# nurturenature/jepsen-tigerbeetle

Measured on NVIDIA H100. Metric: configs explored/sec (time-to-verdict alongside) on 10k-op/32-client bank history, higher is better.
Workload: dtype int64

## Files before the change

### jepsen_tigerbeetle_b200/csrc/jtb_abi.cu

```cuda
#include <algorithm>
#include <chrono>
#include <cstdio>
#include <cstdlib>
#include <cstring>
#include <mutex>
#include <string>
#include <thread>
#include <type_traits>
#include <vector>

#include "jtb_wgl.cuh"
#include "jtb_level.cuh"
#include "jtb_scout.cuh"
#include "jtb_scans.cuh"
#include "jtb_table_bench.cuh"
#include "jtb_partition.cuh"
#include "jtb_monotonic.cuh"
#include "jtb_counter_bounds.cuh"
#include "jtb_transfer_lookups.cuh"
#include "jtb_read_explanations.cuh"
#include "jtb_read_gaps.cuh"

using namespace jtb;

// ... 61 lines not shown
    if (ensure(ctx, b, v.size() * sizeof(T) + 64)) return -1;
    if (!v.empty()) CK(cudaMemcpyAsync(b.p, v.data(), v.size() * sizeof(T), cudaMemcpyHostToDevice, ctx->stream));
    return 0;
}

template <typename F>
int dispatch_model_kw(jtb_ctx* ctx, int kind, int kw, F&& f) {
    using std::integral_constant;
    if (kind == JTB_MODEL_SET) return f(integral_constant<int, JTB_MODEL_SET>(), integral_constant<int, 2>());
    auto by_kw = [&](auto model) -> int {
        switch (kw) {
        case 2: return f(model, integral_constant<int, 2>());
        case 4: return f(model, integral_constant<int, 4>());
        case 8: return f(model, integral_constant<int, 8>());
        }
        ctx->err = "unsupported key width";
        return -1;
    };
    return kind == JTB_MODEL_BANK ? by_kw(integral_constant<int, JTB_MODEL_BANK>())
                                  : by_kw(integral_constant<int, JTB_MODEL_CAS_REGISTER>());
}

template <int MODEL, int KW>
int launch_wgl(jtb_ctx* ctx, const WglParams& p, int neg_ok, int grid, size_t smem) {
    auto k = p.eager_reads ? wgl_search_kernel<MODEL, KW, JTB_CTAS_EAGER, true> : wgl_search_kernel<MODEL, KW, JTB_CTAS_EXACT, false>;
    CK(cudaFuncSetAttribute(k, cudaFuncAttributeMaxDynamicSharedMemorySize, (int)smem));
    k<<<grid, WGL_THREADS, smem, ctx->stream>>>(p, neg_ok);
    CK(cudaGetLastError());
    return 0;
}

template <int MODEL, int KW>
int launch_level(jtb_ctx* ctx, const LvParams& p, int neg_ok, bool eager, int* grid_out) {
    constexpr int EW = KW + (MODEL == JTB_MODEL_BANK ? 4 : 0);
    const bool beam = p.beam_w != 0;
    const size_t smem = (beam ? sizeof(LvScratch<KW, EW, MODEL == JTB_MODEL_BANK, true>)
                              : sizeof(LvScratch<KW, EW, MODEL == JTB_MODEL_BANK, false>)) * LV_WARPS;
    const bool nk = !(MODEL == JTB_MODEL_BANK && !neg_ok);
    const void* k;
#define JTB_LVK(E, N, B) (const void*)level_search_kernel<MODEL, KW, E, (MODEL == JTB_MODEL_BANK ? N : true), B>
    if (beam) k = eager ? (nk ? JTB_LVK(true, true, true) : JTB_LVK(true, false, true)) : (nk ? JTB_LVK(false, true, true) : JTB_LVK(false, false, true));
    else k = eager ? (nk ? JTB_LVK(true, true, false) : JTB_LVK(true, false, false)) : (nk ? JTB_LVK(false, true, false) : JTB_LVK(false, false, false));
#undef JTB_LVK
    CK(cudaFuncSetAttribute(k, cudaFuncAttributeMaxDynamicSharedMemorySize, (int)smem));
    int per_sm = 0;
    CK(cudaOccupancyMaxActiveBlocksPerMultiprocessor(&per_sm, k, LV_THREADS, smem));
    if (per_sm < 1) { ctx->err = "level engine: the kernel does not fit on an SM"; return -1; }
    per_sm = std::min(per_sm, JTB_LV_CTAS);
    const int grid = ctx->opts.search_ctas ? std::min<int>((int)ctx->opts.search_ctas, ctx->n_sms * per_sm) : ctx->n_sms * per_sm;
    if (grid > 1024) { ctx->err = "level engine: more CTAs than barrier release words"; return -1; }
    *grid_out = grid;
    LvParams pp = p;
    void* args[] = {&pp};
    CK(cudaLaunchCooperativeKernel(k, dim3(grid), dim3(LV_THREADS), args, smem, ctx->stream));
    return 0;
}

int search_level(jtb_ctx* ctx, const jtb_model* m, const Prepared& P, int n_shards, const std::vector<int>& searchable,
                 const std::vector<uint64_t>& init_entries, Ctrl& hc, double& kernel_s, uint64_t& configs, uint64_t& probes,
                 uint32_t beam_w = 0) {
    const int KW = P.key_words;
    const bool bank = m->kind == JTB_MODEL_BANK;
    const int EW = KW + (bank ? 4 : 0);
    const bool eager = !(ctx->opts.flags & JTB_OPT_NO_EAGER_READS);
    size_t free_b = 0, total_b = 0;
    CK(cudaMemGetInfo(&free_b, &total_b));
    const size_t reserve = (size_t)4 << 30;
    const size_t avail = ctx->table.cap + ctx->lv_buf[0].cap + ctx->lv_buf[1].cap + (free_b > reserve ? free_b - reserve : 0);
    size_t table_bytes = ctx->opts.table_bytes ? ctx->opts.table_bytes
                         : (getenv("JTB_LV_TABLE_MB") ? (size_t)atoll(getenv("JTB_LV_TABLE_MB")) << 20 : (size_t)1 << 30);
    table_bytes = std::min(table_bytes, avail / 3);
    size_t buf_bytes = getenv("JTB_LV_BUF_MB") ? (size_t)atoll(getenv("JTB_LV_BUF_MB")) << 20 : (size_t)512 << 20;
    buf_bytes = std::max<size_t>(std::min(buf_bytes, avail / 3), init_entries.size() * 8 + 4096);
    auto slots_of = [&](size_t bytes) { uint64_t s = 1; while (s * 2 * KW * 8 <= bytes) s <<= 1; return s; };
    uint64_t table_slots = slots_of(std::max(table_bytes, ctx->table.cap));
    auto ensure_table = [&](uint64_t slots) -> int {
        const void* before = ctx->table.p;
        if (ensure(ctx, ctx->table, slots * KW * 8)) return -1;
        if (ctx->table.p != before) ctx->table_dirty = ~(size_t)0;
        return 0;
    };
    if (ensure_table(table_slots)) return -1;
    if (ensure(ctx, ctx->lv_buf[0], std::max(buf_bytes, ctx->lv_buf[0].cap)) || ensure(ctx, ctx->lv_buf[1], std::max(buf_bytes, ctx->lv_buf[1].cap)) ||
        ensure(ctx, ctx->lv_ctrl, sizeof(LvCtrl)))
        return -1;
    uint64_t buf_cap = std::min(ctx->lv_buf[0].cap, ctx->lv_buf[1].cap) / ((size_t)EW * 8);
    if (beam_w) {
        if (ensure(ctx, ctx->lv_aux[0], buf_cap * 4 + 64) || ensure(ctx, ctx->lv_aux[1], buf_cap * 4 + 64) ||
            ensure(ctx, ctx->lv_beam, sizeof(LvBeam)))
            return -1;
        std::vector<LvBeam> hb(1);
        std::memset(hb.data(), 0, sizeof(LvBeam));
        for (int k = 0; k < 3; ++k)
            for (int s = 0; s < LV_BEAM_SHARDS; ++s) { hb[0].min_crashed[k][s] = 0x7fffffff; hb[0].max_rank[k][s] = -1; }
        for (int s : searchable) { hb[0].min_crashed[0][s] = 0; hb[0].max_rank[0][s] = (int)P.rank_base[s]; }
        CK(cudaMemcpyAsync(ctx->lv_beam.p, hb.data(), sizeof(LvBeam), cudaMemcpyHostToDevice, ctx->stream));
        CK(cudaMemsetAsync(ctx->lv_aux[0].p, 0, init_entries.size() / EW * 4 + 64, ctx->stream));
        CK(cudaStreamSynchronize(ctx->stream));
    }
    CK(cudaMemsetAsync(ctx->table.p, 0, std::min(ctx->table_dirty, (size_t)table_slots * KW * 8), ctx->stream));
    ctx->table_dirty = 0;
    LvCtrl lc;
    std::memset(&lc, 0, sizeof lc);
    lc.n_undecided = (int)searchable.size();
    CK(cudaMemcpyAsync(ctx->lv_ctrl.p, &lc, sizeof lc, cudaMemcpyHostToDevice, ctx->stream));
    CK(cudaMemcpyAsync(ctx->lv_buf[0].p, init_entries.data(), init_entries.size() * 8, cudaMemcpyHostToDevice, ctx->stream));
    LvParams p{};
    p.rows = (const int32_t*)ctx->rows.p;
    p.classes = (const ClassRec*)ctx->classes.p;
    p.cls_inv_pos = (const int32_t*)ctx->cls_inv.p;
    p.ctrl = (LvCtrl*)ctx->lv_ctrl.p;
    p.shard_found = (int*)ctx->found.p;
    p.shard_max_rank = (int*)ctx->maxrank.p;
    p.row_words = P.row_words;
    p.sum_off = P.sum_off;
    p.n_shards = n_shards;
    p.max_configs = ctx->opts.max_configs;
    p.time_budget_ns = (unsigned long long)ctx->opts.time_budget_ms * 1000000ull;
    p.narrow_max = getenv("JTB_LV_NARROW") ? (uint32_t)atoi(getenv("JTB_LV_NARROW")) : (uint32_t)(LV_WARPS * 8);
    p.slots_per_config = getenv("JTB_LV_SPC") ? (uint32_t)std::max(2, atoi(getenv("JTB_LV_SPC"))) : 16u;
    p.min_slots = 1ull << 16;
    std::memset(&p.init, 0, sizeof p.init);
    p.init.n_in = searchable.size();
    p.init.epoch = 1;
    p.init.s_in = 0; p.init.s_out = 1; p.init.s_spare = 2;
    p.init.contig = 1;
    p.init.beam_thr = -1;
    p.init.beam_frac = 1024;
    p.beam_w = beam_w;
    p.aux[0] = (uint32_t*)ctx->lv_aux[0].p;
    p.aux[1] = (uint32_t*)ctx->lv_aux[1].p;
    p.beam = (LvBeam*)ctx->lv_beam.p;
    p.init.win = 0;
    CK(cudaEventRecord(ctx->ev0, ctx->stream));
    int attempts = 0, grid = 0;
    unsigned long long max_window = 0, max_width = 0, narrow_levels = 0, max_probe = 0;
    const double t_begin = now_s();
    for (;;) {
        ++attempts;
// ... 74 lines not shown
        CK(cudaFree(ctx->lv_buf[ii].p));
        ctx->lv_buf[ii] = grown;
        if (ensure(ctx, ctx->lv_buf[ii ^ 1], new_buf)) return -1;
        table_slots = slots_of(new_table);
        if (ensure_table(table_slots)) return -1;
        CK(cudaMemsetAsync(ctx->table.p, 0, (size_t)table_slots * KW * 8, ctx->stream));
        ctx->table_dirty = 0;
        buf_cap = new_buf / ((size_t)EW * 8);
        LvState r = lc.fin;
        r.stop = 0; r.cause = 0; r.boost = 0; r.attempt = 0; r.epoch = 1;
        r.s_in = 0; r.s_out = 1; r.s_spare = 2; r.contig = 1;
        p.init = r;
        const int undecided = lc.n_undecided;
        std::memset(&lc, 0, sizeof lc);
        lc.n_undecided = undecided;
        CK(cudaMemcpyAsync(ctx->lv_ctrl.p, &lc, sizeof lc, cudaMemcpyHostToDevice, ctx->stream));
    }
    CK(cudaEventRecord(ctx->ev1, ctx->stream));
    CK(cudaStreamSynchronize(ctx->stream));
    float ms = 0;
    CK(cudaEventElapsedTime(&ms, ctx->ev0, ctx->ev1));
    kernel_s = ms * 1e-3;
    configs = lc.fin.total;
    std::memset(&hc, 0, sizeof hc);
    hc.stop = lc.fin.stop;
    hc.cause = lc.fin.cause;
    hc.configs = lc.fin.total;
    hc.probes = probes;
    hc.n_undecided = lc.n_undecided;
    unsigned long long* st = ctx->stats;
    st[0] = configs; st[1] = probes; st[2] = lc.fin.level + 1; st[3] = max_width; st[4] = narrow_levels; st[5] = 0;
    st[6] = max_probe; st[7] = max_window; st[8] = (unsigned long long)grid; st[9] = buf_cap;
    st[10] = (unsigned long long)attempts; st[11] = (unsigned long long)(ms * 1e3);
    st[12] += init_entries.size() * 8 + sizeof(LvCtrl) + (size_t)n_shards * 4;
    st[13] = (unsigned long long)attempts * sizeof(LvCtrl) + (size_t)n_shards * 8;
    st[14] = (unsigned long long)attempts;
    st[19] = 1;
    return 0;
}

struct ScoutGuard {
    jtb_ctx* ctx;
    bool active = false;
    explicit ScoutGuard(jtb_ctx* c) : ctx(c) {}
    int stop() {
        if (!active) return 0;
        active = false;
        static const unsigned long long one = 1;
        cudaError_t e = cudaMemcpyAsync((unsigned long long*)ctx->sc_ctl.p + 1, &one, 8, cudaMemcpyHostToDevice, ctx->stream);
        if (e == cudaSuccess) e = cudaStreamSynchronize(ctx->scout_stream);
        if (e != cudaSuccess) { ctx->err = std::string("stopping the scouts: ") + cudaGetErrorString(e); return -1; }
        return 0;
    }
    ~ScoutGuard() { stop(); }
};

template <typename K>
int preload(jtb_ctx* ctx, K kernel) {
    cudaFuncAttributes a;
    CK(cudaFuncGetAttributes(&a, kernel));
    return 0;
}

template <int MODEL, int KW>
int preload_search(jtb_ctx* ctx, bool eager) {
    constexpr int EW = KW + (MODEL == JTB_MODEL_BANK ? 4 : 0);
    int rc = eager ? (preload(ctx, wgl_search_kernel<MODEL, KW, JTB_CTAS_EAGER, true>) | preload(ctx, wgl_scout_kernel<MODEL, KW, true>))
// ... 785 lines not shown
```

### jepsen_tigerbeetle_b200/csrc/jtb_expand.h

```cpp
#pragma once
#include <cstdint>

#include "jtb_prep.h"

#if defined(__CUDACC__)
#define JTB_HD __host__ __device__ __forceinline__
#else
#define JTB_HD inline
#endif

namespace jtb {

constexpr uint64_t XKEY_VALID = 1ull << 63;
constexpr uint32_t XRANK_MASK = 0x1fffffffu;

struct I4 {
    int32_t x, y, z, w;
};

JTB_HD I4 ld_i4(const int32_t* p) {
#if defined(__CUDA_ARCH__)
    const int4 v = __ldg(reinterpret_cast<const int4*>(p));
    return I4{v.x, v.y, v.z, v.w};
#else
// ... 55 lines not shown

    JTB_HD int load_header(const ExpandTables& T) {
        gj = (int)((w[0] >> 32) & XRANK_MASK);
        reg = (int32_t)(uint32_t)w[0];
        row = T.rows + (size_t)gj * T.row_words;
        const I4 h2 = ld_i4(row + 8);
        fr_pos = h2.x; shard = h2.y; gj_end = h2.z; cls_base = h2.w;
        return shard;
    }

    JTB_HD bool read_consistent(const I4& op, const int32_t* cell, uint32_t balhash) const {
        if constexpr (REG) {
            return op.y == JTB_NIL || op.y == reg;
        } else if constexpr (BANK) {
            if ((op.x & OP_HASHED) && (uint32_t)op.z != balhash) return false;
            const I4 lo = ld_i4(cell + 4), hi = ld_i4(cell + 8);
            const int care = op.y;
            bool ok = true;
            ok &= !(care & 1) || bal[0] == lo.x;
            ok &= !(care & 2) || bal[1] == lo.y;
            ok &= !(care & 4) || bal[2] == lo.z;
            ok &= !(care & 8) || bal[3] == lo.w;
            ok &= !(care & 16) || bal[4] == hi.x;
            ok &= !(care & 32) || bal[5] == hi.y;
            ok &= !(care & 64) || bal[6] == hi.z;
            ok &= !(care & 128) || bal[7] == hi.w;
            return ok;
        } else {
            const I4 nc = ld_i4(cell + 4);
            return (w[1] & u64_of(nc.z, nc.w)) == u64_of(nc.x, nc.y);
        }
    }

    JTB_HD void begin(const ExpandTables& T, bool alive) {
        (void)T;
        const I4 h3 = ld_i4(row + 12);
        const I4 h4 = ld_i4(row + 16);
        ncls = h3.x; rslot = h3.y;
        todo = 0; rd_ok = 0; cls_i = ncls;
        if (!alive) return;
        const uint64_t cand = u64_of(h3.z, h3.w) & ~w[1];
        const uint64_t rdm = u64_of(h4.x, h4.y);
        uint64_t rds = cand & rdm;
        uint32_t balhash = 0;
        if constexpr (BANK) {
            if (rds) {
#pragma unroll
                for (int i = 0; i < 8; ++i) balhash += (uint32_t)bal[i] * bank_hash_c(i);
            }
        }
        if constexpr (!SET) {
            const uint64_t fastm = T.sum_off ? (rds & u64_of(h4.z, h4.w)) : 0ull;
            if (fastm) {
                const int32_t* sum = row + T.sum_off;
                const int32_t want = BANK ? (int32_t)balhash : reg;
                uint64_t match = 0;
#if defined(__CUDA_ARCH__)
#pragma unroll 1
#endif
                for (int b = 0; b < 4; ++b) {
                    if (!((fastm >> (16 * b)) & 0xffffull)) continue;
                    uint32_t mm = 0;
#pragma unroll
                    for (int g = 0; g < 4; ++g) {
                        const I4 v = ld_i4(sum + 16 * b + 4 * g);
                        uint32_t m4 = (v.x == want) | ((v.y == want) << 1) | ((v.z == want) << 2) | ((v.w == want) << 3);
                        if constexpr (REG)
                            m4 |= (v.x == JTB_NIL) | ((v.y == JTB_NIL) << 1) | ((v.z == JTB_NIL) << 2) | ((v.w == JTB_NIL) << 3);
                        mm |= m4 << (4 * g);
                    }
                    match |= (uint64_t)mm << (16 * b);
                }
                match &= fastm;
                if constexpr (REG && !EAGER) { rd_ok |= match; match = 0; }
                rds = (rds & ~fastm) | match;
            }
        }
        uint32_t best_inv = 0xffffffffu;
        int best_t = -1;
// ... 122 lines not shown
```

### jepsen_tigerbeetle_b200/csrc/jtb_level.cuh

```cuda
#pragma once
#include "jtb_expand.h"
#include "jtb_wgl.cuh"

namespace jtb {

#ifndef JTB_LV_WARPS
#define JTB_LV_WARPS 8
#endif
#ifndef JTB_LV_CTAS
#define JTB_LV_CTAS 3
#endif
constexpr int LV_WARPS = JTB_LV_WARPS;
constexpr int LV_THREADS = LV_WARPS * 32;
constexpr int LV_STAGE = 64;
constexpr int LV_MAX_PROBE = 128;
constexpr int LV_CLS_WORDS = 8;
constexpr uint64_t LV_TAG_MASK = 0x3full << 56;
constexpr int64_t LV_MAX_RANKS = 1ll << 24;

constexpr int LV_NSEG = 64;
constexpr unsigned LV_F_DECIDED = 1, LV_F_GIVEUP = 2, LV_F_RETRY = 4;

struct LvSeg {
    alignas(128) unsigned long long n;
// ... 34 lines not shown
    unsigned long long max_probe_len, max_width, max_window, narrow_levels, retries, t0, t1;
    LvState fin;
    unsigned long long prof[16];
    unsigned long long prof_cta[1024][2];
    int trace[2048][6];
    alignas(128) LvRelease arrive[1024];
    alignas(128) LvRelease release[1024];
};

struct LvParams {
    const int32_t* rows;
    const ClassRec* classes;
    const int32_t* cls_inv_pos;
    uint64_t* table;
    uint64_t table_slots;
    uint64_t* buf[2];
    uint32_t* aux[2];
    LvBeam* beam;
    uint32_t beam_w;
    uint64_t buf_cap;
    uint64_t seg_cap;
    LvCtrl* ctrl;
    int* shard_found;
    int* shard_max_rank;
    int row_words, sum_off, n_shards;
    unsigned long long max_configs;
    unsigned long long time_budget_ns;
    LvState init;
    uint32_t narrow_max;
    uint32_t slots_per_config;
    uint64_t min_slots;
};

template <int KW, int EW, bool BAL, bool BEAM>
struct LvScratch {
    uint64_t w[32][KW];
    uint64_t todo[32], rd_ok[32];
    uint64_t cls_todo[32][BEAM ? LV_CLS_WORDS : 1];
    int32_t bal[BAL ? 32 : 1][8];
    int32_t hdr[32][6];
    uint32_t start[36];
    uint32_t crashed[BEAM ? 32 : 1];
    uint32_t stage_aux[BEAM ? LV_STAGE : 1];
    uint64_t stage[LV_STAGE][EW];
};

__device__ __forceinline__ int select64(uint64_t m, int k) {
    const uint32_t lo = (uint32_t)m;
    const int c = __popc(lo);
    return k < c ? (int)__fns(lo, 0, k + 1) : 32 + (int)__fns((uint32_t)(m >> 32), 0, k - c + 1);
}

__device__ __forceinline__ void lv_load_state(LvState& dst, const LvState* src) {
    static_assert(sizeof(LvState) % 8 == 0, "LvState is copied as 64-bit words");
    uint64_t* d = reinterpret_cast<uint64_t*>(&dst);
    const uint64_t* q = reinterpret_cast<const uint64_t*>(src);
#pragma unroll
    for (int i = 0; i < (int)(sizeof(LvState) / 8); ++i) d[i] = ldcg64(q + i);
}

template <int KW>
__device__ __forceinline__ int lv_insert(uint64_t* table, uint64_t mask, const uint64_t (&k)[KW], uint64_t tag, int* plen) {
    uint64_t idx = hash_key<KW>(k) & mask;
    const uint64_t mine0 = k[0] | tag;
    for (int i = 0; i < LV_MAX_PROBE; ++i) {
        uint64_t* slot = table + idx * KW;
        K128 cur = ldcg128(slot);
        for (int round = 0; round < 2; ++round) {
            const bool free_slot = !(cur.lo >> 63) || (cur.lo & LV_TAG_MASK) != tag;
            if (!free_slot) break;
            const K128 mine{KW == 2 ? mine0 : (mine0 | KEY_LOCK), k[1]};
            const K128 old = cas128(slot, cur, mine);
            if (old.lo == cur.lo && old.hi == cur.hi) {
                if constexpr (KW > 2) {
#pragma unroll
                    for (int x = 2; x < KW; ++x) slot[x] = k[x];
                    __threadfence();
// ... 94 lines not shown
    return s < p.table_slots ? s : p.table_slots;
}

__device__ __forceinline__ void lv_advance(const LvParams& p, LvState& st, unsigned long long cnt, bool over, unsigned flags) {
    st.attempt++;
    st.epoch = (st.epoch + 1) & 63;
    const int o_in = st.s_in, o_out = st.s_out, o_spare = st.s_spare;
    if (flags & LV_F_GIVEUP) { st.stop = 2; st.cause = (int)(flags >> 8); return; }
    if (flags & LV_F_RETRY) {
        if (st.win >= p.table_slots) { st.stop = 2; st.cause = JTB_CAUSE_TABLE_FULL; return; }
        st.boost++;
        st.win = lv_window(p, st.n_in, st.boost);
        st.s_out = o_spare; st.s_spare = o_out;
        return;
    }
    if (over) { st.stop = 2; st.cause = JTB_CAUSE_TABLE_FULL; return; }
    st.total += cnt;
    if (flags & LV_F_DECIDED) { st.stop = 1; return; }
    if (cnt == 0) { st.stop = 1; return; }
    if (p.max_configs && st.total >= p.max_configs) { st.stop = 2; st.cause = JTB_CAUSE_BUDGET; return; }
    st.level++;
    st.n_in = cnt;
    st.in_idx ^= 1;
    st.contig = 0;
    st.beam_thr = -1;
    st.win = lv_window(p, st.n_in, st.boost);
    st.s_in = o_out; st.s_out = o_spare; st.s_spare = o_in;
}

template <int MODEL, int KW, bool EAGER, bool NEGOK, bool BEAM>
__global__ void __launch_bounds__(LV_THREADS, JTB_LV_CTAS) level_search_kernel(const LvParams p) {
    constexpr bool neg_ok = NEGOK;
    constexpr int CLS_WORDS = BEAM ? LV_CLS_WORDS : 1;
    using L = EntryLayout<MODEL, KW>;
    constexpr int EW = L::EW;
    constexpr bool BAL = L::HAS_BAL;
    constexpr unsigned FULL = 0xffffffffu;
    using Scratch = LvScratch<KW, EW, BAL, BEAM>;
    extern __shared__ __align__(16) unsigned char lv_smem[];
    __shared__ LvState s_state;
    __shared__ unsigned long long s_seg_start[LV_NSEG + 1];
    const int tid = threadIdx.x, lane = tid & 31, warp = tid >> 5;
    const unsigned lt_mask = (1u << lane) - 1;
    Scratch& S = reinterpret_cast<Scratch*>(lv_smem)[warp];
    LvCtrl* ctrl = p.ctrl;
    ExpandTables T;
    T.rows = p.rows; T.classes = p.classes; T.cls_inv_pos = p.cls_inv_pos; T.row_words = p.row_words; T.sum_off = p.sum_off;

    LvState st = p.init;
    unsigned long long bar_gen = 0;
    unsigned long long my_probes = 0;
    int my_max_probe = 0;
    int wit_shard = -1, wit_rank = -1;
    if (blockIdx.x == 0 && tid == 0) ctrl->t0 = globaltimer();
    if (tid <= LV_NSEG) s_seg_start[tid] = tid == 0 ? 0 : st.n_in;
    __syncthreads();

    auto entry_of = [&](const LvState& a, unsigned long long idx, unsigned long long& eidx) -> const uint64_t* {
        int lo = 0, hi = LV_NSEG;
        while (hi - lo > 1) {
            const int mid = (lo + hi) >> 1;
            if (s_seg_start[mid] <= idx) lo = mid; else hi = mid;
        }
        eidx = (unsigned long long)lo * p.seg_cap + (idx - s_seg_start[lo]);
        return p.buf[a.in_idx] + eidx * EW;
    };

    auto run_attempt = [&](const LvState& a, unsigned first_chunk, unsigned chunk_stride) {
        unsigned G = 32, g_log = 5;
        if (a.n_in < 32ull * chunk_stride) {
            const unsigned q = ((unsigned)a.n_in + chunk_stride - 1) / chunk_stride;
            g_log = q <= 1 ? 0 : 32 - __clz(q - 1);
            G = 1u << g_log;
        }
        const unsigned n_chunks = (unsigned)((a.n_in + G - 1) >> g_log);
        if (first_chunk >= n_chunks) return;
        uint64_t* out = p.buf[a.in_idx ^ 1];
        unsigned* res_flags = &ctrl->flags[a.s_out][0];
        const unsigned my_seg = first_chunk % LV_NSEG;
        unsigned long long* my_cnt = &ctrl->seg[a.s_out][my_seg].n;
        uint64_t* my_out = out + (unsigned long long)my_seg * p.seg_cap * EW;
        const uint64_t wmask = a.win - 1;
        const uint64_t tag = (uint64_t)a.epoch << 56;
        unsigned stg_head = 0, stg_tail = 0;
        int bt_shard = -1, bt_min = 0x7fffffff, bt_max = -1;
        auto flush = [&](unsigned n) {
            unsigned long long base = 0;
            if (lane == 0) base = atomicAdd(my_cnt, (unsigned long long)n);
            base = __shfl_sync(FULL, base, 0);
            if (base + n <= p.seg_cap) {
                uint64_t* dst = my_out + base * EW;
                for (unsigned x = lane; x < n * EW; x += 32) {
                    const unsigned e = x / EW, k = x - e * EW;
                    dst[x] = S.stage[(stg_head + e) % LV_STAGE][k];
                }
                if (BEAM && (unsigned)lane < n)
                    p.aux[a.in_idx ^ 1][(unsigned long long)my_seg * p.seg_cap + base + lane] = S.stage_aux[(stg_head + lane) % LV_STAGE];
            }
            stg_head += n;
            __syncwarp();
        };
#ifdef JTB_LV_PROF
        long long tp = clock64();
        if (blockIdx.x == 0 && threadIdx.x == 0) ctrl->prof[8]++;
#endif
        for (unsigned chunk = first_chunk; chunk < n_chunks; chunk += chunk_stride) {
            const unsigned long long idx = (unsigned long long)chunk * G + lane;
            const bool have = (unsigned)lane < G && idx < a.n_in;
            uint64_t todo = 0;
            unsigned n_cls_children = 0;
            {
                Expander<MODEL, KW, EAGER> X;
                X.todo = 0; X.rd_ok = 0; X.ncls = 0; X.cls_i = 0;
                X.fr_pos = 0; X.shard = 0; X.gj_end = 0; X.cls_base = 0; X.rslot = 0;
                if (have) {
                    unsigned long long eidx;
                    const uint64_t* e = entry_of(a, idx, eidx);
                    unsigned crashed = 0;
                    if constexpr (BEAM) crashed = __ldcg(p.aux[a.in_idx] + eidx);
#pragma unroll
                    for (int i = 0; i < KW; ++i) X.w[i] = ldcg64(e + i);
                    if constexpr (BAL) {
#pragma unroll
                        for (int i = 0; i < 4; ++i) {
                            const uint64_t v = ldcg64(e + KW + i);
                            X.bal[2 * i] = (int32_t)(uint32_t)v;
                            X.bal[2 * i + 1] = (int32_t)(uint32_t)(v >> 32);
                        }
                    }
                    const int shard = X.load_header(T);
                    bool alive = !(p.n_shards > 1 && ld_volatile(&p.shard_found[shard]));
                    if constexpr (BEAM) {
                        S.crashed[lane] = crashed & 0xffffu;
                        if (a.beam_thr >= 0) {
                            const int key = (int)(crashed >> 16);
                            alive = alive && (key < a.beam_thr ||
                                              (key == a.beam_thr && (int)((hash_key<KW>(X.w) >> 17) & 1023) < a.beam_frac));
                        }
                    }
                    X.begin(T, alive);
                    todo = X.todo;
#pragma unroll
                    for (int cw = 0; cw < CLS_WORDS; ++cw) S.cls_todo[lane][cw] = 0;
                    if (X.cls_i == 0) {
                        uint64_t cw_bits = 0;
                        for (int ci = 0; ci < X.ncls; ++ci) {
                            const int32_t* q = reinterpret_cast<const int32_t*>(T.classes + X.cls_base + ci);
                            const I4 b = ld_i4(q + 4);
                            const int shift = b.w & 0xff, width = b.w >> 8;
                            uint64_t field = 0;
#pragma unroll
                            for (int i = 1; i < KW; ++i) if (i == b.z) field = X.w[i];
                            const int count = (int)((field >> shift) & ((1ull << width) - 1));
                            if (count < b.y && ld_i32(T.cls_inv_pos + b.x + count) < X.fr_pos) { cw_bits |= 1ull << (ci & 63); ++n_cls_children; }
                            if ((ci & 63) == 63 || ci == X.ncls - 1) { S.cls_todo[lane][ci >> 6] = cw_bits; cw_bits = 0; }
                        }
                    }
#pragma unroll
                    for (int i = 0; i < KW; ++i) S.w[lane][i] = X.w[i];
                    if constexpr (BAL) {
#pragma unroll
                        for (int i = 0; i < 8; ++i) S.bal[lane][i] = X.bal[i];
                    }
                    S.rd_ok[lane] = X.rd_ok;
                    S.hdr[lane][0] = X.fr_pos; S.hdr[lane][1] = X.shard; S.hdr[lane][2] = X.gj_end;
                    S.hdr[lane][3] = X.cls_base; S.hdr[lane][4] = X.rslot; S.hdr[lane][5] = X.ncls;
                }
                S.todo[lane] = todo;
            }
            unsigned c = (unsigned)__popcll(todo) + n_cls_children;
            unsigned incl = c;
#pragma unroll
            for (int o = 1; o < 32; o <<= 1) {
                const unsigned v = __shfl_up_sync(FULL, incl, o);
                if (lane >= o) incl += v;
            }
            LV_PROF(0, tp);
            S.start[lane] = incl - c;
            const unsigned total = __shfl_sync(FULL, incl, 31);
            if (lane == 0) S.start[32] = total;
            __syncwarp();
            for (unsigned g0 = 0; g0 < total; g0 += 32) {
                const unsigned g = g0 + lane;
                const bool act = g < total;
                Child<KW> ch;
                bool is_new = false;
                int owner = 0;
                unsigned child_crashed = 0;
                if (act) {
                    int lo = 0, hi = 32;
                    while (hi - lo > 1) {
                        const int mid = (lo + hi) >> 1;
                        if (S.start[mid] <= g) lo = mid; else hi = mid;
                    }
                    owner = lo;
                    const int k = (int)(g - S.start[owner]);
                    Expander<MODEL, KW, EAGER> Y;
#pragma unroll
                    for (int i = 0; i < KW; ++i) Y.w[i] = S.w[owner][i];
                    if constexpr (BAL && !NEGOK) {
#pragma unroll
                        for (int i = 0; i < 8; ++i) Y.bal[i] = S.bal[owner][i];
                    }
                    Y.rd_ok = S.rd_ok[owner];
                    Y.gj = (int)((Y.w[0] >> 32) & XRANK_MASK);
                    Y.reg = (int32_t)(uint32_t)Y.w[0];
                    Y.row = T.rows + (size_t)Y.gj * T.row_words;
                    Y.fr_pos = S.hdr[owner][0]; Y.shard = S.hdr[owner][1]; Y.gj_end = S.hdr[owner][2];
                    Y.cls_base = S.hdr[owner][3]; Y.rslot = S.hdr[owner][4]; Y.ncls = S.hdr[owner][5];
                    const uint64_t otodo = S.todo[owner];
                    const int ns = __popcll(otodo);
                    bool ok;
                    int t_slot = 0;
                    if constexpr (BEAM) child_crashed = S.crashed[owner] + (k >= ns ? 1u : 0u);
                    if (k < ns) { t_slot = select64(otodo, k); ok = Y.child_slot(T, t_slot, neg_ok, ch, true); }
                    else {
                        int kk = k - ns, cw = 0;
                        for (; cw < CLS_WORDS - 1; ++cw) {
                            const int pc = __popcll(S.cls_todo[owner][cw]);
                            if (kk < pc) break;
                            kk -= pc;
                        }
                        ok = Y.child_class(T, cw * 64 + select64(S.cls_todo[owner][cw], kk), neg_ok, ch);
                    }
                    if (ok) {
                        if (ch.done) {
                            if (atomicExch(&p.shard_found[Y.shard], 1) == 0) {
                                if (atomicSub(&ctrl->n_undecided, 1) == 1) atomicOr(res_flags, LV_F_DECIDED);
                            }
                        } else {
                            int plen;
                            const int r = lv_insert<KW>(p.table, wmask, ch.w, tag, &plen);
                            my_probes++;
                            my_max_probe = max(my_max_probe, plen);
                            if (r < 0) atomicOr(res_flags, LV_F_RETRY);
                            is_new = r == 1;
                            if constexpr (BAL) {
                                if (is_new && ch.d < 0) Y.load_transfer(t_slot, ch);
                            }
                            if (is_new && ch.cgj > Y.gj && (wit_shard != Y.shard || wit_rank < ch.cgj)) {
                                wit_shard = Y.shard; wit_rank = ch.cgj;
                                atomicMax(&p.shard_max_rank[Y.shard], ch.cgj);
                            }
                            if (BEAM && is_new) {
                                LvBeam* bm = p.beam;
                                const int key = lv_beam_key((int)child_crashed, __ldcg(&bm->min_crashed[a.s_in][Y.shard]), ch.cgj,
                                                            __ldcg(&bm->max_rank[a.s_in][Y.shard]));
                                atomicAdd(&bm->hist[a.s_out][key], 1u);
                                child_crashed = min(child_crashed, 0xffffu) | ((unsigned)key << 16);
                                if (bt_shard != Y.shard) { bt_shard = Y.shard; bt_min = 0x7fffffff; bt_max = -1; }
                                const int cc = (int)(child_crashed & 0xffffu);
                                if (cc < bt_min) { bt_min = cc; atomicMin(&bm->min_crashed[a.s_out][Y.shard], bt_min); }
                                if (ch.cgj > bt_max) { bt_max = ch.cgj; atomicMax(&bm->max_rank[a.s_out][Y.shard], bt_max); }
                            }
                        }
                    }
                }
                const unsigned newm = __ballot_sync(FULL, is_new);
                if (newm) {
                    if (is_new) {
                        uint64_t* e = S.stage[(stg_tail + __popc(newm & lt_mask)) % LV_STAGE];
                        if constexpr (BEAM) S.stage_aux[(stg_tail + __popc(newm & lt_mask)) % LV_STAGE] = child_crashed;
#pragma unroll
                        for (int i = 0; i < KW; ++i) e[i] = ch.w[i];
                        if constexpr (BAL) {
                            int32_t b[8];
#pragma unroll
                            for (int i = 0; i < 8; ++i) b[i] = S.bal[owner][i];
                            if (ch.amt) {
#pragma unroll
                                for (int i = 0; i < 8; ++i) {
                                    if (i == ch.d) b[i] -= ch.amt;
                                    if (i == ch.c) b[i] += ch.amt;
                                }
                            }
#pragma unroll
                            for (int i = 0; i < 4; ++i) e[KW + i] = u64_of(b[2 * i], b[2 * i + 1]);
                        }
                    }
                    stg_tail += __popc(newm);
                    __syncwarp();
                    if (stg_tail - stg_head >= 32) flush(32);
                }
            }
            __syncwarp();
            LV_PROF(1, tp);
        }
        if (stg_tail != stg_head) flush(stg_tail - stg_head);
        LV_PROF(2, tp);
    };

    auto collect = [&](LvState& a) {
        if (warp == 0) {
            const unsigned long long c0 = ld_volatile(&ctrl->seg[a.s_out][lane].n);
            const unsigned long long c1 = ld_volatile(&ctrl->seg[a.s_out][lane + 32].n);
            unsigned fl = 0;
            if (lane == 0) fl = *(volatile unsigned*)&ctrl->flags[a.s_out][0];
            const bool over = c0 > p.seg_cap || c1 > p.seg_cap;
            unsigned long long i0 = c0, i1 = c1;
#pragma unroll
            for (int o = 1; o < 32; o <<= 1) {
                const unsigned long long v0 = __shfl_up_sync(FULL, i0, o), v1 = __shfl_up_sync(FULL, i1, o);
                if (lane >= o) { i0 += v0; i1 += v1; }
            }
            const unsigned long long t0 = __shfl_sync(FULL, i0, 31);
            const unsigned long long t1 = __shfl_sync(FULL, i1, 31);
            const bool any_over = __any_sync(FULL, over);
            LvState nx = a;
            if (lane == 0) lv_advance(p, nx, t0 + t1, any_over, fl);
            int thr = -1, frac = 1024;
            if constexpr (BEAM) {
// ... 159 lines not shown
```

### jepsen_tigerbeetle_b200/csrc/jtb_prep.cpp

```cpp
#include "jtb_prep.h"

#include <algorithm>
#include <climits>
#include <cstring>
#include <map>
#include <tuple>
#include <unordered_map>

namespace jtb {
namespace {

struct HOp {
    int inv_pos, ret_pos;
    int inv_ev, ret_ev;
    bool crashed, dropped;
    int slot, rank;
    int cls;
};

struct ShardTmp {
    std::vector<HOp> ops;
    std::vector<int> rets;
    int S = 0;
    std::vector<std::vector<int>> cls_members;
// ... 324 lines not shown
    out.rows.assign((size_t)out.n_ranks * RW, 0);
    out.ret_index.assign((size_t)out.n_ranks, -1);
    for (int s = 0; s < n_shards; ++s) {
        ShardTmp& t = tmp[s];
        const int R = (int)t.rets.size();
        if (R == 0) continue;
        const int64_t base = out.rank_base[s];
        const int32_t op_base = (int32_t)out.ops.size();
        std::vector<int32_t> gid(t.ops.size(), -1);
        std::vector<int32_t> op_inv_pos;
        std::vector<int32_t> op_read_bal;
        for (int i = 0; i < (int)t.ops.size(); ++i) {
            if (t.ops[i].crashed) continue;
            gid[i] = (int32_t)out.ops.size();
            out.ops.push_back(resolve(h, m, t.ops[i].ret_ev, out));
            op_inv_pos.push_back(t.ops[i].inv_pos);
            op_read_bal.push_back(out.ops.back().w);
            const bool transfer = m->kind == JTB_MODEL_BANK && (out.ops.back().x & 0xff) == JTB_F_TRANSFER;
            if (!transfer) out.ops.back().w = t.ops[i].inv_pos;
        }
        const int32_t cls_base = (int32_t)out.classes.size();
        for (size_t c = 0; c < t.cls_members.size(); ++c) {
            ClassRec cr;
            cr.op = resolve(h, m, t.ops[t.cls_rep[c]].inv_ev, out);
            cr.first = (int32_t)out.cls_inv_pos.size();
            cr.n = (int32_t)t.cls_members[c].size();
            cr.word = field[s][c].first;
            cr.shift_width = field[s][c].second;
            for (int i : t.cls_members[c]) out.cls_inv_pos.push_back(t.ops[i].inv_pos);
            out.classes.push_back(cr);
        }
        std::vector<int32_t> cur(out.S_pad, -1);
        size_t oi = 0;
        for (int j = 0; j < R; ++j) {
            const HOp& ro = t.ops[t.rets[j]];
            while (oi < t.ops.size() && t.ops[oi].inv_pos < ro.ret_pos) {
                if (!t.ops[oi].crashed) cur[t.ops[oi].slot] = gid[oi];
                ++oi;
            }
            int32_t* row = &out.rows[(size_t)(base + j) * RW];
            uint8_t* nxt = reinterpret_cast<uint8_t*>(row);
            for (int k = 0; k < 32; ++k)
                nxt[k] = (j + 1 + k < R) ? (uint8_t)t.ops[t.rets[j + 1 + k]].slot : (uint8_t)0xFF;
            row[8] = ro.ret_pos;
            row[9] = s;
            row[10] = (int32_t)(base + R);
            row[11] = cls_base;
            row[12] = (int32_t)t.cls_members.size();
            row[13] = ro.slot;
            for (int sl = 0; sl < out.S_pad; ++sl) {
                int32_t* cell = row + ROW_EXTRA + sl * SW;
                if (cur[sl] < 0) { cell[0] = OP_EMPTY; continue; }
                const OpRec& rec = out.ops[cur[sl]];
                cell[0] = rec.x; cell[1] = rec.y; cell[2] = rec.z; cell[3] = rec.w;
                if (m->kind == JTB_MODEL_BANK) {
                    if ((rec.x & 0xff) == JTB_F_READ)
                        std::memcpy(cell + 4, &out.read_bal[(size_t)op_read_bal[cur[sl] - op_base] * JTB_MAX_ACCOUNTS],
                                    8 * sizeof(int32_t));
                    else
                        cell[4] = op_inv_pos[cur[sl] - op_base];
                }
            }
            out.ret_index[base + j] = h->index[ro.ret_ev];
            cur[ro.slot] = -1;
        }
        if (m->kind == JTB_MODEL_SET) {
            std::vector<int32_t> fr_pos(R);
            for (int j = 0; j < R; ++j) fr_pos[j] = t.ops[t.rets[j]].ret_pos;
            if (!build_set_tables(h, t, gid, base, field[s], fr_pos, out)) {
                out.shard_cause[s] = JTB_CAUSE_TOO_WIDE;
            }
        }
        for (int j = 0; j < R; ++j) {
            int32_t* row = &out.rows[(size_t)(base + j) * RW];
            uint64_t occ = 0, rd = 0, fast = 0;
            for (int sl = 0; sl < out.S_pad; ++sl) {
                const int32_t* cell = row + ROW_EXTRA + sl * SW;
                const int32_t x = cell[0];
                if (x < 0 || (x & OP_IMPOSSIBLE)) continue;
                occ |= 1ull << sl;
                if ((x & 0xff) != JTB_F_READ) continue;
                rd |= 1ull << sl;
                if (m->kind == JTB_MODEL_BANK) {
                    if (x & OP_HASHED) { fast |= 1ull << sl; row[out.sum_off + sl] = cell[2]; }
                } else if (m->kind != JTB_MODEL_SET) {
                    fast |= 1ull << sl;
                    row[out.sum_off + sl] = cell[1];
                }
            }
            std::memcpy(row + 14, &occ, 8);
            std::memcpy(row + 16, &rd, 8);
            std::memcpy(row + 18, &fast, 8);
        }
    }
    {
// ... 13 lines not shown
```

### jepsen_tigerbeetle_b200/csrc/jtb_prep.h

```cpp
#pragma once
#include <cstdint>
#include <string>
#include <vector>

#include "../../include/jtb_check.h"

namespace jtb {

struct OpRec {
    int32_t x, y, z, w;
};
constexpr int OP_IMPOSSIBLE = 1 << 8;
constexpr int OP_HASHED = 1 << 9;
#if defined(__CUDACC__)
__host__ __device__
#endif
constexpr uint32_t bank_hash_c(int i) {
    return i == 0 ? 0x9E3779B1u : i == 1 ? 0x85EBCA77u : i == 2 ? 0xC2B2AE3Du : i == 3 ? 0x27D4EB2Fu :
           i == 4 ? 0x165667B1u : i == 5 ? 0xD3A2646Du : i == 6 ? 0xFD7046C5u : 0xB55A4F09u;
}

struct ClassRec {
    OpRec op;
    int32_t first;
    int32_t n;
    int32_t word;
    int32_t shift_width;
};

constexpr int ROW_EXTRA = 20;
inline int slot_words(int model) { return model == JTB_MODEL_BANK ? 12 : model == JTB_MODEL_SET ? 8 : 4; }
constexpr int OP_EMPTY = -1;

struct Prepared {
    int S_pad = 32;
    int key_words = 2;
    int model = 0;
    int64_t n_ranks = 0;
    int row_words = 0;
    int sum_off = 0;
    std::vector<int32_t> rows;
    std::vector<OpRec> ops;
    std::vector<int32_t> read_bal;
    std::vector<ClassRec> classes;
    std::vector<int32_t> cls_inv_pos;
    std::vector<int64_t> rank_base;
    std::vector<int32_t> ret_index;
    std::vector<int32_t> shard_cause;
    std::vector<int32_t> max_classes;
    int max_nc = 0;
    double mean_open = 0;
    std::string error;
};

bool prepare(const jtb_history* h, const jtb_model* m, Prepared& out);

}
```

Before: 3.487 billion.

## Recompute bank balances from row prefix sums instead of storing them per frontier entry

Frontier entries in the level search no longer carry four extra words of account balances. Instead each row stores prefix balances computed on the host, and the kernel rebuilds a configuration's balances by applying linearized transfers and class counts. This shrinks frontier buffer traffic and staging shared memory for the bank model. The cost is extra per-expansion arithmetic and row or class loads, and it relies on uint32 wraparound arithmetic matching the old results.

```diff
diff --git a/jepsen_tigerbeetle_b200/csrc/jtb_abi.cu b/jepsen_tigerbeetle_b200/csrc/jtb_abi.cu
--- a/jepsen_tigerbeetle_b200/csrc/jtb_abi.cu
+++ b/jepsen_tigerbeetle_b200/csrc/jtb_abi.cu
@@ -117,11 +117,10 @@
 
 template <int MODEL, int KW>
 int launch_level(jtb_ctx* ctx, const LvParams& p, int neg_ok, bool eager, int* grid_out) {
-    constexpr int EW = KW + (MODEL == JTB_MODEL_BANK ? 4 : 0);
     const bool beam = p.beam_w != 0;
-    const size_t smem = (beam ? sizeof(LvScratch<KW, EW, MODEL == JTB_MODEL_BANK, true>)
-                              : sizeof(LvScratch<KW, EW, MODEL == JTB_MODEL_BANK, false>)) * LV_WARPS;
     const bool nk = !(MODEL == JTB_MODEL_BANK && !neg_ok);
+    const size_t smem = (beam ? (nk ? sizeof(LvScratch<KW, false, true>) : sizeof(LvScratch<KW, true, true>))
+                              : (nk ? sizeof(LvScratch<KW, false, false>) : sizeof(LvScratch<KW, true, false>))) * LV_WARPS;
     const void* k;
 #define JTB_LVK(E, N, B) (const void*)level_search_kernel<MODEL, KW, E, (MODEL == JTB_MODEL_BANK ? N : true), B>
     if (beam) k = eager ? (nk ? JTB_LVK(true, true, true) : JTB_LVK(true, false, true)) : (nk ? JTB_LVK(false, true, true) : JTB_LVK(false, false, true));
@@ -146,8 +145,14 @@
                  uint32_t beam_w = 0) {
     const int KW = P.key_words;
     const bool bank = m->kind == JTB_MODEL_BANK;
-    const int EW = KW + (bank ? 4 : 0);
     const bool eager = !(ctx->opts.flags & JTB_OPT_NO_EAGER_READS);
+    const int EW = KW;
+    std::vector<uint64_t> init_keys;
+    {
+        const size_t in_ew = (size_t)KW + (bank ? 4 : 0);
+        for (size_t i = 0; i + in_ew <= init_entries.size(); i += in_ew)
+            init_keys.insert(init_keys.end(), init_entries.begin() + i, init_entries.begin() + i + KW);
+    }
     size_t free_b = 0, total_b = 0;
     CK(cudaMemGetInfo(&free_b, &total_b));
     const size_t reserve = (size_t)4 << 30;
@@ -156,7 +161,7 @@
                          : (getenv("JTB_LV_TABLE_MB") ? (size_t)atoll(getenv("JTB_LV_TABLE_MB")) << 20 : (size_t)1 << 30);
     table_bytes = std::min(table_bytes, avail / 3);
     size_t buf_bytes = getenv("JTB_LV_BUF_MB") ? (size_t)atoll(getenv("JTB_LV_BUF_MB")) << 20 : (size_t)512 << 20;
-    buf_bytes = std::max<size_t>(std::min(buf_bytes, avail / 3), init_entries.size() * 8 + 4096);
+    buf_bytes = std::max<size_t>(std::min(buf_bytes, avail / 3), init_keys.size() * 8 + 4096);
     auto slots_of = [&](size_t bytes) { uint64_t s = 1; while (s * 2 * KW * 8 <= bytes) s <<= 1; return s; };
     uint64_t table_slots = slots_of(std::max(table_bytes, ctx->table.cap));
     auto ensure_table = [&](uint64_t slots) -> int {
@@ -180,7 +185,7 @@
             for (int s = 0; s < LV_BEAM_SHARDS; ++s) { hb[0].min_crashed[k][s] = 0x7fffffff; hb[0].max_rank[k][s] = -1; }
         for (int s : searchable) { hb[0].min_crashed[0][s] = 0; hb[0].max_rank[0][s] = (int)P.rank_base[s]; }
         CK(cudaMemcpyAsync(ctx->lv_beam.p, hb.data(), sizeof(LvBeam), cudaMemcpyHostToDevice, ctx->stream));
-        CK(cudaMemsetAsync(ctx->lv_aux[0].p, 0, init_entries.size() / EW * 4 + 64, ctx->stream));
+        CK(cudaMemsetAsync(ctx->lv_aux[0].p, 0, init_keys.size() / EW * 4 + 64, ctx->stream));
         CK(cudaStreamSynchronize(ctx->stream));
     }
     CK(cudaMemsetAsync(ctx->table.p, 0, std::min(ctx->table_dirty, (size_t)table_slots * KW * 8), ctx->stream));
@@ -189,7 +194,7 @@
     std::memset(&lc, 0, sizeof lc);
     lc.n_undecided = (int)searchable.size();
     CK(cudaMemcpyAsync(ctx->lv_ctrl.p, &lc, sizeof lc, cudaMemcpyHostToDevice, ctx->stream));
-    CK(cudaMemcpyAsync(ctx->lv_buf[0].p, init_entries.data(), init_entries.size() * 8, cudaMemcpyHostToDevice, ctx->stream));
+    CK(cudaMemcpyAsync(ctx->lv_buf[0].p, init_keys.data(), init_keys.size() * 8, cudaMemcpyHostToDevice, ctx->stream));
     LvParams p{};
     p.rows = (const int32_t*)ctx->rows.p;
     p.classes = (const ClassRec*)ctx->classes.p;
@@ -330,7 +335,7 @@
     st[0] = configs; st[1] = probes; st[2] = lc.fin.level + 1; st[3] = max_width; st[4] = narrow_levels; st[5] = 0;
     st[6] = max_probe; st[7] = max_window; st[8] = (unsigned long long)grid; st[9] = buf_cap;
     st[10] = (unsigned long long)attempts; st[11] = (unsigned long long)(ms * 1e3);
-    st[12] += init_entries.size() * 8 + sizeof(LvCtrl) + (size_t)n_shards * 4;
+    st[12] += init_keys.size() * 8 + sizeof(LvCtrl) + (size_t)n_shards * 4;
     st[13] = (unsigned long long)attempts * sizeof(LvCtrl) + (size_t)n_shards * 8;
     st[14] = (unsigned long long)attempts;
     st[19] = 1;
diff --git a/jepsen_tigerbeetle_b200/csrc/jtb_expand.h b/jepsen_tigerbeetle_b200/csrc/jtb_expand.h
--- a/jepsen_tigerbeetle_b200/csrc/jtb_expand.h
+++ b/jepsen_tigerbeetle_b200/csrc/jtb_expand.h
@@ -111,7 +111,43 @@
         }
     }
 
-    JTB_HD void begin(const ExpandTables& T, bool alive) {
+    JTB_HD void rebuild_balances(const ExpandTables& T) {
+        const I4 p0 = ld_i4(row + ROW_PREFIX_BAL), p1 = ld_i4(row + ROW_PREFIX_BAL + 4);
+        uint32_t b[8] = {(uint32_t)p0.x, (uint32_t)p0.y, (uint32_t)p0.z, (uint32_t)p0.w,
+                         (uint32_t)p1.x, (uint32_t)p1.y, (uint32_t)p1.z, (uint32_t)p1.w};
+        auto apply = [&](const I4& op, uint32_t times) {
+            if ((op.x & 0xff) != JTB_F_TRANSFER) return;
+            const uint32_t amt = (uint32_t)op.y * times;
+#pragma unroll
+            for (int i = 0; i < 8; ++i) b[i] += (i == op.w ? amt : 0u) - (i == op.z ? amt : 0u);
+        };
+        const I4 h3 = ld_i4(row + 12);
+        uint64_t lin = w[1] & u64_of(h3.z, h3.w);
+        while (lin) {
+            I4 op[4];
+#pragma unroll
+            for (int k = 0; k < 4; ++k) {
+                const int t = lin ? ctz64(lin) : -1;
+                lin &= lin - 1;
+                op[k] = t >= 0 ? ld_i4(row + ROW_EXTRA + t * SW) : I4{0, 0, 0, 0};
+            }
+#pragma unroll
+            for (int k = 0; k < 4; ++k) apply(op[k], 1u);
+        }
+        for (int ci = 0; ci < h3.x; ++ci) {
+            const int32_t* q = reinterpret_cast<const int32_t*>(T.classes + cls_base + ci);
+            const I4 cb = ld_i4(q + 4);
+            uint64_t field = 0;
+#pragma unroll
+            for (int i = 1; i < KW; ++i) if (i == cb.z) field = w[i];
+            const uint32_t count = (uint32_t)((field >> (cb.w & 0xff)) & ((1ull << (cb.w >> 8)) - 1));
+            if (count) apply(ld_i4(q), count);
+        }
+#pragma unroll
+        for (int i = 0; i < 8; ++i) bal[i] = (int32_t)b[i];
+    }
+
+    JTB_HD void begin(const ExpandTables& T, bool alive, bool lazy_bal = false) {
         (void)T;
         const I4 h3 = ld_i4(row + 12);
         const I4 h4 = ld_i4(row + 16);
@@ -124,6 +160,7 @@
         uint32_t balhash = 0;
         if constexpr (BANK) {
             if (rds) {
+                if (lazy_bal) rebuild_balances(T);
 #pragma unroll
                 for (int i = 0; i < 8; ++i) balhash += (uint32_t)bal[i] * bank_hash_c(i);
             }
diff --git a/jepsen_tigerbeetle_b200/csrc/jtb_level.cuh b/jepsen_tigerbeetle_b200/csrc/jtb_level.cuh
--- a/jepsen_tigerbeetle_b200/csrc/jtb_level.cuh
+++ b/jepsen_tigerbeetle_b200/csrc/jtb_level.cuh
@@ -90,7 +90,7 @@
     uint64_t min_slots;
 };
 
-template <int KW, int EW, bool BAL, bool BEAM>
+template <int KW, bool BAL, bool BEAM>
 struct LvScratch {
     uint64_t w[32][KW];
     uint64_t todo[32], rd_ok[32];
@@ -100,7 +100,7 @@
     uint32_t start[36];
     uint32_t crashed[BEAM ? 32 : 1];
     uint32_t stage_aux[BEAM ? LV_STAGE : 1];
-    uint64_t stage[LV_STAGE][EW];
+    uint64_t stage[LV_STAGE][KW];
 };
 
 __device__ __forceinline__ int select64(uint64_t m, int k) {
@@ -261,11 +261,10 @@
 __global__ void __launch_bounds__(LV_THREADS, JTB_LV_CTAS) level_search_kernel(const LvParams p) {
     constexpr bool neg_ok = NEGOK;
     constexpr int CLS_WORDS = BEAM ? LV_CLS_WORDS : 1;
-    using L = EntryLayout<MODEL, KW>;
-    constexpr int EW = L::EW;
-    constexpr bool BAL = L::HAS_BAL;
+    constexpr bool BANK = MODEL == JTB_MODEL_BANK;
+    constexpr bool BAL = BANK && !NEGOK;
     constexpr unsigned FULL = 0xffffffffu;
-    using Scratch = LvScratch<KW, EW, BAL, BEAM>;
+    using Scratch = LvScratch<KW, BAL, BEAM>;
     extern __shared__ __align__(16) unsigned char lv_smem[];
     __shared__ LvState s_state;
     __shared__ unsigned long long s_seg_start[LV_NSEG + 1];
@@ -292,7 +291,7 @@
             if (s_seg_start[mid] <= idx) lo = mid; else hi = mid;
         }
         eidx = (unsigned long long)lo * p.seg_cap + (idx - s_seg_start[lo]);
-        return p.buf[a.in_idx] + eidx * EW;
+        return p.buf[a.in_idx] + eidx * KW;
     };
 
     auto run_attempt = [&](const LvState& a, unsigned first_chunk, unsigned chunk_stride) {
@@ -308,7 +307,7 @@
         unsigned* res_flags = &ctrl->flags[a.s_out][0];
         const unsigned my_seg = first_chunk % LV_NSEG;
         unsigned long long* my_cnt = &ctrl->seg[a.s_out][my_seg].n;
-        uint64_t* my_out = out + (unsigned long long)my_seg * p.seg_cap * EW;
+        uint64_t* my_out = out + (unsigned long long)my_seg * p.seg_cap * KW;
         const uint64_t wmask = a.win - 1;
         const uint64_t tag = (uint64_t)a.epoch << 56;
         unsigned stg_head = 0, stg_tail = 0;
@@ -318,9 +317,9 @@
             if (lane == 0) base = atomicAdd(my_cnt, (unsigned long long)n);
             base = __shfl_sync(FULL, base, 0);
             if (base + n <= p.seg_cap) {
-                uint64_t* dst = my_out + base * EW;
-                for (unsigned x = lane; x < n * EW; x += 32) {
-                    const unsigned e = x / EW, k = x - e * EW;
+                uint64_t* dst = my_out + base * KW;
+                for (unsigned x = lane; x < n * KW; x += 32) {
+                    const unsigned e = x / KW, k = x - e * KW;
                     dst[x] = S.stage[(stg_head + e) % LV_STAGE][k];
                 }
                 if (BEAM && (unsigned)lane < n)
@@ -349,14 +348,6 @@
                     if constexpr (BEAM) crashed = __ldcg(p.aux[a.in_idx] + eidx);
 #pragma unroll
                     for (int i = 0; i < KW; ++i) X.w[i] = ldcg64(e + i);
-                    if constexpr (BAL) {
-#pragma unroll
-                        for (int i = 0; i < 4; ++i) {
-                            const uint64_t v = ldcg64(e + KW + i);
-                            X.bal[2 * i] = (int32_t)(uint32_t)v;
-                            X.bal[2 * i + 1] = (int32_t)(uint32_t)(v >> 32);
-                        }
-                    }
                     const int shard = X.load_header(T);
                     bool alive = !(p.n_shards > 1 && ld_volatile(&p.shard_found[shard]));
                     if constexpr (BEAM) {
@@ -367,7 +358,10 @@
                                               (key == a.beam_thr && (int)((hash_key<KW>(X.w) >> 17) & 1023) < a.beam_frac));
                         }
                     }
-                    X.begin(T, alive);
+                    if constexpr (BAL) {
+                        if (alive) X.rebuild_balances(T);
+                    }
+                    X.begin(T, alive, BANK && !BAL);
                     todo = X.todo;
 #pragma unroll
                     for (int cw = 0; cw < CLS_WORDS; ++cw) S.cls_todo[lane][cw] = 0;
@@ -427,7 +421,7 @@
                     Expander<MODEL, KW, EAGER> Y;
 #pragma unroll
                     for (int i = 0; i < KW; ++i) Y.w[i] = S.w[owner][i];
-                    if constexpr (BAL && !NEGOK) {
+                    if constexpr (BAL) {
 #pragma unroll
                         for (int i = 0; i < 8; ++i) Y.bal[i] = S.bal[owner][i];
                     }
@@ -464,9 +458,6 @@
                             my_max_probe = max(my_max_probe, plen);
                             if (r < 0) atomicOr(res_flags, LV_F_RETRY);
                             is_new = r == 1;
-                            if constexpr (BAL) {
-                                if (is_new && ch.d < 0) Y.load_transfer(t_slot, ch);
-                            }
                             if (is_new && ch.cgj > Y.gj && (wit_shard != Y.shard || wit_rank < ch.cgj)) {
                                 wit_shard = Y.shard; wit_rank = ch.cgj;
                                 atomicMax(&p.shard_max_rank[Y.shard], ch.cgj);
@@ -492,20 +483,6 @@
                         if constexpr (BEAM) S.stage_aux[(stg_tail + __popc(newm & lt_mask)) % LV_STAGE] = child_crashed;
 #pragma unroll
                         for (int i = 0; i < KW; ++i) e[i] = ch.w[i];
-                        if constexpr (BAL) {
-                            int32_t b[8];
-#pragma unroll
-                            for (int i = 0; i < 8; ++i) b[i] = S.bal[owner][i];
-                            if (ch.amt) {
-#pragma unroll
-                                for (int i = 0; i < 8; ++i) {
-                                    if (i == ch.d) b[i] -= ch.amt;
-                                    if (i == ch.c) b[i] += ch.amt;
-                                }
-                            }
-#pragma unroll
-                            for (int i = 0; i < 4; ++i) e[KW + i] = u64_of(b[2 * i], b[2 * i + 1]);
-                        }
                     }
                     stg_tail += __popc(newm);
                     __syncwarp();
diff --git a/jepsen_tigerbeetle_b200/csrc/jtb_prep.cpp b/jepsen_tigerbeetle_b200/csrc/jtb_prep.cpp
--- a/jepsen_tigerbeetle_b200/csrc/jtb_prep.cpp
+++ b/jepsen_tigerbeetle_b200/csrc/jtb_prep.cpp
@@ -380,6 +380,8 @@
         }
         std::vector<int32_t> cur(out.S_pad, -1);
         size_t oi = 0;
+        uint32_t prefix_bal[JTB_MAX_ACCOUNTS];
+        for (int i = 0; i < JTB_MAX_ACCOUNTS; ++i) prefix_bal[i] = (uint32_t)m->init_balance[i];
         for (int j = 0; j < R; ++j) {
             const HOp& ro = t.ops[t.rets[j]];
             while (oi < t.ops.size() && t.ops[oi].inv_pos < ro.ret_pos) {
@@ -409,6 +411,14 @@
                         cell[4] = op_inv_pos[cur[sl] - op_base];
                 }
             }
+            if (m->kind == JTB_MODEL_BANK) {
+                for (int i = 0; i < JTB_MAX_ACCOUNTS; ++i) row[ROW_PREFIX_BAL + i] = (int32_t)prefix_bal[i];
+                const OpRec& rec = out.ops[cur[ro.slot]];
+                if ((rec.x & 0xff) == JTB_F_TRANSFER && !(rec.x & OP_IMPOSSIBLE)) {
+                    prefix_bal[rec.z] -= (uint32_t)rec.y;
+                    prefix_bal[rec.w] += (uint32_t)rec.y;
+                }
+            }
             out.ret_index[base + j] = h->index[ro.ret_ev];
             cur[ro.slot] = -1;
         }
diff --git a/jepsen_tigerbeetle_b200/csrc/jtb_prep.h b/jepsen_tigerbeetle_b200/csrc/jtb_prep.h
--- a/jepsen_tigerbeetle_b200/csrc/jtb_prep.h
+++ b/jepsen_tigerbeetle_b200/csrc/jtb_prep.h
@@ -28,7 +28,8 @@
     int32_t shift_width;
 };
 
-constexpr int ROW_EXTRA = 20;
+constexpr int ROW_PREFIX_BAL = 20;
+constexpr int ROW_EXTRA = 28;
 inline int slot_words(int model) { return model == JTB_MODEL_BANK ? 12 : model == JTB_MODEL_SET ? 8 : 4; }
 constexpr int OP_EMPTY = -1;
 
```

Measured after the change: 3.567 billion (median of 6 runs). 2.3% higher.
